# openMVG/openMVG

Hardware: AMD Instinct MI355X
Metric: descriptor pairs/s (brute-force L2 2-NN + ratio matching) (higher is better)
Workload: dtype i8 (int32 accumulate); 1 GPU; 1000 images x 2000 SIFT-like uint8x128 descriptors, exhaustive pairs (499500 image pairs, 499500 on rank 0), ratio 0.8; parallelism=pair-sharded x1, no collective

## Files before the change

### include/mvgx.h

```cpp
#ifndef MVGX_H_
#define MVGX_H_

#include <stddef.h>
#include <stdint.h>

#ifdef __cplusplus
extern "C" {
#endif

#define MVGX_OK 0
#define MVGX_ERR_ARG 1
#define MVGX_ERR_HIP 2
#define MVGX_ERR_NODEV 3
#define MVGX_ERR_STATE 4
#define MVGX_ERR_UNSUPPORTED 5
#define MVGX_ERR_NUMERIC 6
#define MVGX_ERR_STRUCTURE 7

const char* mvgx_last_error(void);
int mvgx_device_count(int* count);
int mvgx_abi_version(void);


typedef struct mvgx_match_ctx mvgx_match_ctx;
// ... 10 lines not shown
  uint32_t kernel_vgprs;
  uint32_t variant;
} mvgx_match_stats;

int mvgx_match_create(int device, mvgx_match_ctx** out);
int mvgx_match_create_multi(const int* devices, int n_devices, mvgx_match_ctx** out);
int mvgx_match_destroy(mvgx_match_ctx* ctx);

int mvgx_match_set_option(mvgx_match_ctx* ctx, const char* key, int64_t value);

int mvgx_match_set_regions(mvgx_match_ctx* ctx, const uint8_t* const* desc_rows, const uint32_t* n_desc,
                           uint32_t n_images, uint32_t dim);

int mvgx_match_set_regions_device(mvgx_match_ctx* ctx, const void* d_desc_concat, const uint32_t* n_desc,
                                  uint32_t n_images, uint32_t dim);

int mvgx_match_run(mvgx_match_ctx* ctx, const uint32_t* pairs_IJ, uint64_t n_pairs, float ratio_sq,
                   mvgx_match_stats* stats );

typedef int (*mvgx_match_batch_sink)(void* user, uint64_t first_pair, uint32_t n_pairs, const uint32_t* offsets,
                                     const uint32_t* ij);
int mvgx_match_run_stream(mvgx_match_ctx* ctx, const uint32_t* pairs_IJ, uint64_t n_pairs, float ratio_sq,
                          mvgx_match_batch_sink sink, void* user, mvgx_match_stats* stats );

int mvgx_match_results(mvgx_match_ctx* ctx, const uint64_t** offsets, const uint32_t** ij);

int mvgx_match_pairs_u8_l2(const uint8_t* const* desc_rows, const uint32_t* n_desc, uint32_t n_images,
                           uint32_t dim, const uint32_t* pairs_IJ, uint64_t n_pairs, float ratio_sq,
                           int device, mvgx_match_sink sink, void* user);

typedef struct mvgx_hamming_ctx mvgx_hamming_ctx;
int mvgx_hamming_create(int device, mvgx_hamming_ctx** out);
int mvgx_hamming_destroy(mvgx_hamming_ctx* ctx);
int mvgx_hamming_set_option(mvgx_hamming_ctx* ctx, const char* key , int64_t value);
int mvgx_hamming_set_regions(mvgx_hamming_ctx* ctx, const uint8_t* const* desc_rows, const uint32_t* n_desc,
                             uint32_t n_images, uint32_t desc_bytes);
int mvgx_hamming_run(mvgx_hamming_ctx* ctx, const uint32_t* pairs_IJ, uint64_t n_pairs, float dist_ratio,
                     mvgx_match_stats* stats );
int mvgx_hamming_results(mvgx_hamming_ctx* ctx, const uint64_t** offsets, const uint32_t** ij);

typedef struct mvgx_l2f_ctx mvgx_l2f_ctx;
int mvgx_l2f_create(int device, mvgx_l2f_ctx** out);
int mvgx_l2f_destroy(mvgx_l2f_ctx* ctx);
int mvgx_l2f_set_option(mvgx_l2f_ctx* ctx, const char* key , int64_t value);
int mvgx_l2f_set_regions(mvgx_l2f_ctx* ctx, const float* const* desc_rows, const uint32_t* n_desc, uint32_t n_images,
                         uint32_t dim);
// ... 273 lines not shown
```

### openmvg_amd/_capi.py

```python
import ctypes as C
import os

_HERE = os.path.dirname(os.path.abspath(__file__))
LIB_PATH = os.environ.get("MVGX_LIB_PATH") or os.path.join(_HERE, "lib", "libmvgx_hip.so")

MVGX_OK = 0
MVGX_ERR_ARG, MVGX_ERR_HIP, MVGX_ERR_NODEV, MVGX_ERR_STATE, MVGX_ERR_UNSUPPORTED, MVGX_ERR_NUMERIC, MVGX_ERR_STRUCTURE = 1, 2, 3, 4, 5, 6, 7
MVGX_BA_MAX_INTR_PARAMS = 8


class MvgxError(RuntimeError):
    def __init__(self, code, msg):
        super().__init__(f"mvgx error {code}: {msg}")
        self.code = code


class MatchStats(C.Structure):
    _fields_ = [
        ("n_pairs", C.c_uint64),
        ("n_desc_pairs", C.c_uint64),
        ("n_matches", C.c_uint64),
        ("n_kernel_launches", C.c_uint64),
        ("kernel_ms", C.c_double),
        ("total_ms", C.c_double),
# ... 117 lines not shown
class ResectionOptions(C.Structure):
    _fields_ = [("solver", C.c_int32), ("max_iteration", C.c_uint32), ("error_max", C.c_double), ("waves_ahead", C.c_uint32),
                ("global_above", C.c_uint32)]


class ResectionStats(C.Structure):
    _fields_ = [("n_problems", C.c_uint64), ("n_iterations", C.c_uint64), ("n_models", C.c_uint64), ("kernel_ms", C.c_double),
                ("total_ms", C.c_double)]


PROTOTYPES = {
    "mvgx_last_error": (C.c_char_p, []),
    "mvgx_device_count": (C.c_int, [C.POINTER(C.c_int)]),
    "mvgx_abi_version": (C.c_int, []),
    "mvgx_match_create": (C.c_int, [C.c_int, C.POINTER(C.c_void_p)]),
    "mvgx_match_create_multi": (C.c_int, [C.POINTER(C.c_int), C.c_int, C.POINTER(C.c_void_p)]),
    "mvgx_match_destroy": (C.c_int, [C.c_void_p]),
    "mvgx_match_set_option": (C.c_int, [C.c_void_p, C.c_char_p, C.c_int64]),
    "mvgx_match_set_regions": (C.c_int, [C.c_void_p, C.POINTER(C.c_void_p), C.POINTER(C.c_uint32), C.c_uint32, C.c_uint32]),
    "mvgx_match_set_regions_device": (C.c_int, [C.c_void_p, C.c_void_p, C.POINTER(C.c_uint32), C.c_uint32, C.c_uint32]),
    "mvgx_match_run": (C.c_int, [C.c_void_p, C.c_void_p, C.c_uint64, C.c_float, C.POINTER(MatchStats)]),
    "mvgx_match_run_stream": (C.c_int, [C.c_void_p, C.c_void_p, C.c_uint64, C.c_float, MATCH_BATCH_SINK, C.c_void_p,
                                        C.POINTER(MatchStats)]),
    "mvgx_match_results": (C.c_int, [C.c_void_p, C.POINTER(C.POINTER(C.c_uint64)), C.POINTER(C.POINTER(C.c_uint32))]),
    "mvgx_match_pairs_u8_l2": (C.c_int, [C.POINTER(C.c_void_p), C.POINTER(C.c_uint32), C.c_uint32, C.c_uint32, C.c_void_p,
                                          C.c_uint64, C.c_float, C.c_int, MATCH_SINK, C.c_void_p]),
    "mvgx_hamming_create": (C.c_int, [C.c_int, C.POINTER(C.c_void_p)]),
    "mvgx_hamming_destroy": (C.c_int, [C.c_void_p]),
    "mvgx_hamming_set_option": (C.c_int, [C.c_void_p, C.c_char_p, C.c_int64]),
    "mvgx_hamming_set_regions": (C.c_int, [C.c_void_p, C.POINTER(C.c_void_p), C.POINTER(C.c_uint32), C.c_uint32, C.c_uint32]),
    "mvgx_hamming_run": (C.c_int, [C.c_void_p, C.c_void_p, C.c_uint64, C.c_float, C.POINTER(MatchStats)]),
    "mvgx_hamming_results": (C.c_int, [C.c_void_p, C.POINTER(C.POINTER(C.c_uint64)), C.POINTER(C.POINTER(C.c_uint32))]),
    "mvgx_l2f_create": (C.c_int, [C.c_int, C.POINTER(C.c_void_p)]),
    "mvgx_l2f_destroy": (C.c_int, [C.c_void_p]),
    "mvgx_l2f_set_option": (C.c_int, [C.c_void_p, C.c_char_p, C.c_int64]),
    "mvgx_l2f_set_regions": (C.c_int, [C.c_void_p, C.POINTER(C.c_void_p), C.POINTER(C.c_uint32), C.c_uint32, C.c_uint32]),
    "mvgx_l2f_run": (C.c_int, [C.c_void_p, C.c_void_p, C.c_uint64, C.c_float, C.POINTER(MatchStats)]),
    "mvgx_l2f_results": (C.c_int, [C.c_void_p, C.POINTER(C.POINTER(C.c_uint64)), C.POINTER(C.POINTER(C.c_uint32))]),
    "mvgx_l2u8_create": (C.c_int, [C.c_int, C.POINTER(C.c_void_p)]),
    "mvgx_l2u8_destroy": (C.c_int, [C.c_void_p]),
    "mvgx_l2u8_set_option": (C.c_int, [C.c_void_p, C.c_char_p, C.c_int64]),
    "mvgx_l2u8_set_regions": (C.c_int, [C.c_void_p, C.POINTER(C.c_void_p), C.POINTER(C.c_uint32), C.c_uint32, C.c_uint32]),
    "mvgx_l2u8_run": (C.c_int, [C.c_void_p, C.c_void_p, C.c_uint64, C.c_float, C.POINTER(MatchStats)]),
    "mvgx_l2u8_results": (C.c_int, [C.c_void_p, C.POINTER(C.POINTER(C.c_uint64)), C.POINTER(C.POINTER(C.c_uint32))]),
    "mvgx_cascade_create": (C.c_int, [C.c_int, C.POINTER(C.c_void_p)]),
    "mvgx_cascade_destroy": (C.c_int, [C.c_void_p]),
# ... 98 lines not shown
```

### openmvg_amd/csrc/mvgx_match.hip

```cpp
#include <hip/hip_runtime.h>

#include <algorithm>
#include <atomic>
#include <climits>
#include <condition_variable>
#include <cstdint>
#include <cstdlib>
#include <cstring>
#include <functional>
#include <mutex>
#include <string>
#include <thread>
#include <vector>

#include "mvgx_buffers.h"
#include "mvgx_common.h"
#include "mvgx_match_batch.h"

namespace {

using mvgx::DevBuf;
using mvgx::PinnedBuf;
using mvgx::set_error;

// ... 1175 lines not shown
      const uint32_t* dbr = reinterpret_cast<const uint32_t*>(rowsI + (size_t)i * kDim);
      int d = 0;
#pragma unroll
      for (int k = 0; k < 32; ++k) {
        const uint32_t x = qv[k], y = dbr[k];
#pragma unroll
        for (int bb = 0; bb < 4; ++bb) {
          const int df = (int)((x >> (8 * bb)) & 0xFF) - (int)((y >> (8 * bb)) & 0xFF);
          d += df * df;
        }
      }
      if (d < d0) { d1 = d0; d0 = d; i0 = i; }
      else if (d < d1) { d1 = d; }
    }
    const bool ok = __int2float_rn(d0) < __fmul_rn(p.ratio_sq, __int2float_rn(d1));
    p.best[(size_t)wk.x * p.qstride + p.rowpos[p.img_row_off[J] + q]] = ok ? i0 : kNoMatch;
    if (ok) atomicAdd(&p.count[wk.x], 1u);
  }
}


}

struct mvgx_match_ctx {
  int device = 0;
  hipStream_t stream = nullptr;
  hipEvent_t ev_total0 = nullptr, ev_total1 = nullptr;
  int variant = 4;
  int filter_shape = 16;
  int stage = 3;
  int profile = 0;
  int64_t batch_pairs = 1 << 15;
  int keep_host_results = 1;
  int overlap = 1;
  int verify_alone = 0;
  int debug_filter = 0;
  int stream_hold = 0;
  int pinned_stream = 1;
  uint32_t n_images = 0;
  uint32_t total_tiles = 0;
  uint32_t max_tiles_pad = 0;
  uint32_t qstride = 0;
  std::vector<uint32_t> h_n, h_tile_off, h_ntiles;
  std::vector<uint32_t> h_qtile_off;
  std::vector<uint64_t> h_row_off;
  DevBuf<uint8_t> d_rows;
  bool rows_owned = true;
  const uint8_t* d_rows_view = nullptr;
  DevBuf<int8_t> d_tiles, d_rows_slot, d_qtiles;
  DevBuf<int> d_rconst, d_cinit, d_qnorm, d_rownorm, d_qtnorm;
  DevBuf<uint64_t> d_row_off;
  DevBuf<uint32_t> d_tile_off, d_qtile_off, d_n, d_ntiles, d_perm, d_rowpos, d_neven, d_err;
  struct Slot {
    hipStream_t stream = nullptr;
    hipEvent_t ev_scan = nullptr;
    hipEvent_t ev_filter = nullptr;
    DevBuf<uint2> d_pairs, d_work, d_ij;
    DevBuf<uint4> d_work8, d_work8h;
    DevBuf<uint32_t> d_best, d_count, d_offsets;
    DevBuf<int2> d_cd;
    PinnedBuf<uint2> hp_pairs, hp_work;
    PinnedBuf<uint4> hp_work8, hp_work8h;
    PinnedBuf<uint32_t> hp_offsets;
    uint64_t p0 = 0;
    uint32_t nb = 0;
    hipEvent_t ev_copy = nullptr;
    PinnedBuf<uint32_t> hp_ij[2];
    std::vector<uint32_t> h_off_out[2];
    int out_set = 0;
    uint64_t out_p0 = 0;
    uint32_t out_nb = 0;
  } slot[2];
  struct Results {
    std::vector<uint64_t> offsets;
    PinnedBuf<uint32_t> ij;
    size_t ij_n = 0;
  } results[2];
  int cur = 0;
  int double_buffer = 0;
  std::vector<hipEvent_t> ev_pool;
  std::vector<mvgx_match_ctx*> children;
};

namespace {

enum WorkList { kListItems16 = 0, kListItems8h = 1, kListRecords = 2 };
using MatchKernel = void (*)(MatchParams);
struct KernelForm {
// ... 37 lines not shown
    for (uint32_t qt = 0; qt < c->h_ntiles[J]; qt += kBlockQTiles) out[n++] = make_uint2(k, qt);
  }
  return n;
}
uint32_t build_items8h(const mvgx_match_ctx* c, const uint32_t* ij, uint32_t nb, uint4* out) {
  uint32_t n = 0;
  for (uint32_t k = 0; k < nb; ++k) {
    const uint32_t I = ij[2 * k], J = ij[2 * k + 1];
    if (!pair_has_work(c, I, J)) continue;
    for (uint32_t qt = 0; qt < c->h_ntiles[J]; qt += kBlockQTilesH) {
      out[2 * n] = make_uint4(k, qt, c->h_tile_off[I], c->h_tile_off[J]);
      out[2 * n + 1] = make_uint4(c->h_ntiles[I], c->h_tile_off[J + 1] - c->h_tile_off[J], 0, 0);
      ++n;
    }
  }
  return n;
}
uint32_t build_records(const mvgx_match_ctx* c, const uint32_t* ij, uint32_t nb, uint4* out) {
  const mvgx_records::ImageTables im{c->h_n.data(), c->h_tile_off.data(), c->h_ntiles.data(), c->h_qtile_off.data()};
  return mvgx_records::build_block_records(im, ij, nb, reinterpret_cast<uint32_t*>(out));
}

template <typename T>
int upload_list(DevBuf<T>& d, const PinnedBuf<T>& h, size_t n, hipStream_t stream) {
  const int rc = d.ensure(std::max<size_t>(n, 1));
  if (rc) return rc;
  if (n) MVGX_HIP(hipMemcpyAsync(d.p, h.p, n * sizeof(T), hipMemcpyHostToDevice, stream));
  return MVGX_OK;
}

int prep_regions(mvgx_match_ctx* c) {
  const uint32_t n_images = c->n_images;
  c->h_tile_off.assign(n_images + 1, 0);
  c->h_row_off.assign(n_images + 1, 0);
  c->h_ntiles.assign(n_images + 1, 0);
  c->h_qtile_off.assign(n_images + 1, 0);
  uint32_t max_n = 0;
  for (uint32_t k = 0; k < n_images; ++k) {
    c->h_row_off[k + 1] = c->h_row_off[k] + c->h_n[k];
    c->h_qtile_off[k + 1] = c->h_qtile_off[k] + (c->h_n[k] + kTileRows - 1) / kTileRows;
    max_n = std::max(max_n, c->h_n[k]);
  }
  const uint64_t total_rows = c->h_row_off[n_images];
  int rc;
  if ((rc = c->d_row_off.ensure(n_images + 1))) return rc;
  if ((rc = c->d_tile_off.ensure(n_images + 1))) return rc;
  if ((rc = c->d_qtile_off.ensure(n_images + 1))) return rc;
  if ((rc = c->d_n.ensure(n_images + 1))) return rc;
// ... 172 lines not shown
}

int mvgx_match_set_option(mvgx_match_ctx* c, const char* key, int64_t value) {
  MVGX_REQUIRE(c && key, MVGX_ERR_ARG, "mvgx_match_set_option: NULL argument");
  if (strcmp(key, "pinned_results") && strcmp(key, "double_buffer_results") && strcmp(key, "keep_host_results"))
    for (mvgx_match_ctx* child : c->children) {
      const int rc = mvgx_match_set_option(child, key, value);
      if (rc) return rc;
    }
  if (!strcmp(key, "variant")) {
    MVGX_REQUIRE(value >= 0 && value <= 4, MVGX_ERR_ARG, "variant must be 0..4");
    c->variant = (int)value;
  } else if (!strcmp(key, "filter_shape")) {
    MVGX_REQUIRE(value == 16 || value == 17 || value == 32, MVGX_ERR_ARG, "filter_shape must be 16, 17 (16x16x64, three workgroups per CU) or 32");
    c->filter_shape = (int)value;
  } else if (!strcmp(key, "stage")) {
    MVGX_REQUIRE(value >= 1 && value <= 3, MVGX_ERR_ARG, "stage must be 1..3");
    c->stage = (int)value;
  } else if (!strcmp(key, "profile")) {
    c->profile = value < 0 ? 0 : (int)std::min<int64_t>(value, 2);
  } else if (!strcmp(key, "batch_pairs")) {
    MVGX_REQUIRE(value >= 1 && value <= (1 << 20), MVGX_ERR_ARG, "batch_pairs must be in [1, 2^20]");
    c->batch_pairs = value;
  } else if (!strcmp(key, "keep_host_results")) {
    c->keep_host_results = value != 0;
  } else if (!strcmp(key, "overlap")) {
    c->overlap = value != 0;
  } else if (!strcmp(key, "verify_alone")) {
    c->verify_alone = value != 0;
  } else if (!strcmp(key, "debug_filter")) {
    MVGX_REQUIRE(value == 0 || value == 8 || value == 16, MVGX_ERR_ARG,
                 "debug_filter must be 0, 8 or 16 (the epilogue forms of l2_filter_kernel: window fold, both partitions per chain, "
                 "window fold with a single-buffered initialiser)");
    c->debug_filter = (int)value;
  } else if (!strcmp(key, "stream_hold")) {
    c->stream_hold = value != 0;
  } else if (!strcmp(key, "pinned_stream")) {
    c->pinned_stream = value != 0;
  } else if (!strcmp(key, "stream_reserve")) {
    MVGX_REQUIRE(value >= 0 && value <= (int64_t)1 << 31, MVGX_ERR_ARG, "stream_reserve: words per buffer in [0, 2^31]");
    if (c->pinned_stream && value > 0) {
      MVGX_HIP(hipSetDevice(c->device));
      for (auto& sl : c->slot)
        for (int set = 0; set < (c->stream_hold ? 2 : 1); ++set) {
          PinnedBuf<uint32_t>& hb = sl.hp_ij[set];
          if (!hb.p) hb.pageable = false;
// ... 56 lines not shown
}

int mvgx_match_set_regions_device(mvgx_match_ctx* c, const void* d_desc_concat, const uint32_t* n_desc,
                                  uint32_t n_images, uint32_t dim) {
  MVGX_REQUIRE(c && n_desc && (d_desc_concat || n_images == 0), MVGX_ERR_ARG,
               "mvgx_match_set_regions_device: NULL argument");
  MVGX_REQUIRE(dim == kDim, MVGX_ERR_UNSUPPORTED, "descriptor length %u unsupported (device path is 128-D uint8)", dim);
  MVGX_REQUIRE(c->children.empty(), MVGX_ERR_UNSUPPORTED, "mvgx_match_set_regions_device: a device pointer belongs to one device; "
               "use mvgx_match_set_regions on a multi-device context");
  MVGX_HIP(hipSetDevice(c->device));
  c->n_images = n_images;
  c->h_n.assign(n_desc, n_desc + n_images);
  c->rows_owned = false;
  c->d_rows_view = static_cast<const uint8_t*>(d_desc_concat);
  return prep_regions(c);
}

}

namespace {

struct BatchFeed {
  const uint32_t* pairs_IJ = nullptr;
  uint64_t n_pairs = 0, B = 1;
  std::atomic<uint64_t> next{0};
  std::atomic<int> stop{0};
  bool take(uint64_t& p0, uint32_t& nb) {
    if (stop.load(std::memory_order_relaxed)) return false;
    p0 = next.fetch_add(B);
    if (p0 >= n_pairs) return false;
    nb = (uint32_t)std::min<uint64_t>(B, n_pairs - p0);
    return true;
  }
};

using BatchSink = std::function<int(uint64_t p0, uint32_t nb, const uint32_t* offsets, const uint32_t* ij)>;

int run_device(mvgx_match_ctx* c, BatchFeed& feed, float ratio_sq, const BatchSink* sink, mvgx_match_stats& st) {
  const uint32_t* pairs_IJ = feed.pairs_IJ;
  MVGX_HIP(hipSetDevice(c->device));
  mvgx_match_ctx::Results& res = c->results[c->cur];
  memset(&st, 0, sizeof(st));
  st.variant = (uint32_t)c->variant;
  size_t n_ev = 0;
  int rc;

  MVGX_HIP(hipEventRecord(c->ev_total0, c->slot[0].stream));

  const KernelForm form = resolve_form(c);
  auto issue = [&](mvgx_match_ctx::Slot& sl, mvgx_match_ctx::Slot* prev, uint64_t p0, uint32_t nb) -> int {
    int rc;
    hipStream_t stream = sl.stream;
    sl.p0 = p0; sl.nb = nb;
    const uint32_t* ij = pairs_IJ + 2 * p0;
    if ((rc = sl.hp_pairs.ensure(nb))) return rc;
    for (uint32_t k = 0; k < nb; ++k) {
      const uint32_t I = ij[2 * k], J = ij[2 * k + 1];
      sl.hp_pairs.p[k] = make_uint2(I, J);
      if (!pair_has_work(c, I, J)) continue;
      st.n_pairs += 1;
      st.n_desc_pairs += (uint64_t)c->h_n[I] * c->h_n[J];
    }
    const size_t max_items16 = (size_t)nb * std::max<uint32_t>(1, (c->max_tiles_pad + kBlockQTiles - 1) / kBlockQTiles);
    uint32_t n_list[3] = {0, 0, 0};
    if (form.reads(kListItems16)) {
      if ((rc = sl.hp_work.ensure(max_items16))) return rc;
      n_list[kListItems16] = build_items16(c, ij, nb, sl.hp_work.p);
    }
    if (form.reads(kListItems8h)) {
      if ((rc = sl.hp_work8h.ensure(max_items16 * 4))) return rc;
      n_list[kListItems8h] = build_items8h(c, ij, nb, sl.hp_work8h.p);
    }
    if (form.reads(kListRecords)) {
      if ((rc = sl.hp_work8.ensure(max_items16 * kRecQuads))) return rc;
      n_list[kListRecords] = build_records(c, ij, nb, sl.hp_work8.p);
    }
    const uint32_t n_filter = n_list[form.list], n_verify = n_list[form.verify_list];
    if ((rc = sl.d_pairs.ensure(nb))) return rc;
    if ((rc = sl.d_best.ensure((size_t)nb * c->qstride))) return rc;
    if (form.verify && (rc = sl.d_cd.ensure((size_t)nb * c->qstride))) return rc;
    if ((rc = sl.d_count.ensure(nb))) return rc;
    if ((rc = sl.d_offsets.ensure((size_t)nb + 1))) return rc;
    if ((rc = sl.hp_offsets.ensure((size_t)nb + 1))) return rc;
    MVGX_HIP(hipMemcpyAsync(sl.d_pairs.p, sl.hp_pairs.p, nb * sizeof(uint2), hipMemcpyHostToDevice, stream));
    if (form.reads(kListItems16) && (rc = upload_list(sl.d_work, sl.hp_work, n_list[kListItems16], stream))) return rc;
    if (form.reads(kListItems8h) && (rc = upload_list(sl.d_work8h, sl.hp_work8h, (size_t)n_list[kListItems8h] * 2, stream))) return rc;
    if (form.reads(kListRecords) && (rc = upload_list(sl.d_work8, sl.hp_work8, (size_t)n_list[kListRecords] * kRecQuads, stream))) return rc;
    MVGX_HIP(hipMemsetAsync(sl.d_count.p, 0, nb * sizeof(uint32_t), stream));

    MatchParams mp;
    mp.tiles = c->d_tiles.p; mp.rows_slot = c->d_rows_slot.p; mp.rconst = c->d_rconst.p; mp.cinit = c->d_cinit.p; mp.qnorm = c->d_qnorm.p;
    mp.perm = c->d_perm.p; mp.rowpos = c->d_rowpos.p; mp.qtiles = c->d_qtiles.p; mp.qtnorm = c->d_qtnorm.p;
    mp.rows_u8 = c->d_rows_view; mp.img_row_off = c->d_row_off.p;
    mp.img_tile_off = c->d_tile_off.p; mp.img_n = c->d_n.p; mp.img_ntiles = c->d_ntiles.p;
    mp.cd = sl.d_cd.p; mp.img_neven = c->d_neven.p; mp.errflag = c->d_err.p;
    mp.pairs = sl.d_pairs.p; mp.work = sl.d_work.p; mp.work8 = sl.d_work8.p; mp.work8h = sl.d_work8h.p; mp.n_work = n_filter;
    mp.best = sl.d_best.p; mp.count = sl.d_count.p; mp.qstride = c->qstride; mp.ratio_sq = ratio_sq;

    if (prev) MVGX_HIP(hipStreamWaitEvent(stream, prev->ev_filter, 0));
    if (n_filter) {
      hipEvent_t e0 = nullptr, e1 = nullptr;
      if (c->profile) {
        e0 = get_event(c, n_ev++); e1 = get_event(c, n_ev++);
        MVGX_REQUIRE(e0 && e1, MVGX_ERR_HIP, "hipEventCreate failed");
        MVGX_HIP(hipEventRecord(e0, stream));
      }
      hipLaunchKernelGGL(form.filter, dim3(n_filter), dim3(256), form.lds_bytes, stream, mp);
      MVGX_HIP(hipGetLastError());
      if (c->profile) MVGX_HIP(hipEventRecord(e1, stream));
      if (!c->verify_alone) MVGX_HIP(hipEventRecord(sl.ev_filter, stream));
// ... 16 lines not shown
    uint32_t* const d_offsets = sl.d_offsets.p;
    hipLaunchKernelGGL(scan_counts_kernel, dim3(1), dim3(1024), 0, stream, mp.count, nb, d_offsets);
    MVGX_HIP(hipGetLastError());
    MVGX_HIP(hipMemcpyAsync(sl.hp_offsets.p, sl.d_offsets.p, ((size_t)nb + 1) * sizeof(uint32_t), hipMemcpyDeviceToHost, stream));
    MVGX_HIP(hipEventRecord(sl.ev_scan, stream));
    return MVGX_OK;
  };
  auto finish = [&](mvgx_match_ctx::Slot& sl) -> int {
    int rc;
    MVGX_HIP(hipEventSynchronize(sl.ev_scan));
    const uint32_t nb = sl.nb;
    const uint64_t p0 = sl.p0;
    const uint32_t total = sl.hp_offsets.p[nb];
    if (sink) {
      if (c->stream_hold) sl.out_set ^= 1;
      sl.h_off_out[sl.out_set].assign(sl.hp_offsets.p, sl.hp_offsets.p + nb + 1);
    } else {
      const uint64_t base = res.offsets[p0];
      for (uint32_t k = 0; k <= nb; ++k) res.offsets[p0 + k] = base + sl.hp_offsets.p[k];
    }
    sl.out_p0 = p0; sl.out_nb = nb;
    st.n_matches += total;
    if (total) {
      if ((rc = sl.d_ij.ensure(total))) return rc;
      hipStream_t stream = sl.stream;
      const uint32_t *d_best = sl.d_best.p, *d_offsets = sl.d_offsets.p;
      const uint2* d_pairs = sl.d_pairs.p;
      uint2* d_ij = sl.d_ij.p;
      hipLaunchKernelGGL(compact_matches_kernel, dim3((nb + 3) / 4), dim3(256), 0, stream, d_best, d_offsets, d_pairs, c->d_n.p,
                         c->d_row_off.p, form.dense_slots ? nullptr : c->d_rowpos.p, nb, c->qstride, d_ij);
      MVGX_HIP(hipGetLastError());
      if (sink) {
        PinnedBuf<uint32_t>& hb = sl.hp_ij[sl.out_set];
        if (!hb.p) hb.pageable = !c->pinned_stream;
        if ((size_t)total * 2 > hb.cap) { hb.release(); if ((rc = hb.grow_keep(std::max<size_t>((size_t)total * 3, 4u << 20), 0))) return rc; }
        MVGX_HIP(hipMemcpyAsync(hb.p, sl.d_ij.p, (size_t)total * sizeof(uint2), hipMemcpyDeviceToHost, sl.stream));
      } else if (c->keep_host_results) {
        const size_t old = res.ij_n;
        if (old + (size_t)total * 2 > res.ij.cap)
          for (auto& o : c->slot) MVGX_HIP(hipStreamSynchronize(o.stream));
        if ((rc = res.ij.grow_keep(old + (size_t)total * 2, old))) return rc;
        res.ij_n = old + (size_t)total * 2;
        MVGX_HIP(hipMemcpyAsync(res.ij.p + old, sl.d_ij.p, (size_t)total * sizeof(uint2),
                                hipMemcpyDeviceToHost, sl.stream));
      }
    }
    if (sink) MVGX_HIP(hipEventRecord(sl.ev_copy, sl.stream));
    return MVGX_OK;
  };
  auto deliver = [&](mvgx_match_ctx::Slot& sl) -> int {
    MVGX_HIP(hipEventSynchronize(sl.ev_copy));
    if (feed.stop.load()) return MVGX_OK;
    if ((*sink)(sl.out_p0, sl.out_nb, sl.h_off_out[sl.out_set].data(), sl.hp_ij[sl.out_set].p)) feed.stop.store(1);
    return MVGX_OK;
  };
  uint64_t nbatch = 0, p0 = 0;
  uint32_t nb = 0;
  while (feed.take(p0, nb)) {
    mvgx_match_ctx::Slot& cur = c->slot[nbatch & 1];
    mvgx_match_ctx::Slot* prev = nbatch ? &c->slot[(nbatch - 1) & 1] : nullptr;
    if (!c->overlap) {
      if ((rc = issue(cur, nullptr, p0, nb)) || (rc = finish(cur))) return rc;
      MVGX_HIP(hipStreamSynchronize(cur.stream));
      if (sink && (rc = deliver(cur))) return rc;
      ++nbatch;
      continue;
    }
    if ((rc = issue(cur, prev, p0, nb))) return rc;
    if (prev && (rc = finish(*prev))) return rc;
    if (sink && nbatch >= 2 && (rc = deliver(cur))) return rc;
    ++nbatch;
  }
  if (c->overlap && nbatch) {
    mvgx_match_ctx::Slot& last = c->slot[(nbatch - 1) & 1];
    if (sink && nbatch >= 2 && (rc = deliver(c->slot[nbatch & 1]))) return rc;
    if ((rc = finish(last))) return rc;
    if (sink && (rc = deliver(last))) return rc;
  }
  for (auto& sl : c->slot) MVGX_HIP(hipStreamSynchronize(sl.stream));
  MVGX_HIP(hipEventRecord(c->ev_total1, c->slot[0].stream));
  MVGX_HIP(hipEventSynchronize(c->ev_total1));
  float ms = 0.f;
  MVGX_HIP(hipEventElapsedTime(&ms, c->ev_total0, c->ev_total1));
  st.total_ms = ms;
  if (form.verify) {
    uint32_t flags[2] = {0, 0};
    MVGX_HIP(hipMemcpy(flags, c->d_err.p, 2 * sizeof(uint32_t), hipMemcpyDeviceToHost));
    (void)hipMemset(c->d_err.p, 0, 2 * sizeof(uint32_t));
    const uint32_t nerr = flags[0];
    st.kernel_vgprs = flags[1];
    if (nerr) {
// ... 85 lines not shown
  MVGX_REQUIRE(c && (pairs_IJ || n_pairs == 0), MVGX_ERR_ARG, "%s: NULL argument", who);
  const mvgx_match_ctx* r = c->children.empty() ? c : c->children[0];
  MVGX_REQUIRE(r->d_rows_view != nullptr || r->n_images == 0, MVGX_ERR_STATE, "%s before set_regions", who);
  const int rc = check_ratio(ratio_sq, "ratio_sq");
  return rc ? rc : check_pairs_in_range(pairs_IJ, n_pairs, r->n_images, who);
}

uint64_t batch_size(const mvgx_match_ctx* c) {
  return batch_size(c->batch_pairs, (c->children.empty() ? c : c->children[0])->qstride);
}

}

extern "C" {

int mvgx_match_run(mvgx_match_ctx* c, const uint32_t* pairs_IJ, uint64_t n_pairs, float ratio_sq,
                   mvgx_match_stats* stats) {
  int rc = check_run_args(c, pairs_IJ, n_pairs, ratio_sq, "mvgx_match_run");
  if (rc) return rc;
  if (c->double_buffer) c->cur ^= 1;
  mvgx_match_ctx::Results& res = c->results[c->cur];
  res.offsets.assign(n_pairs + 1, 0);
  res.ij_n = 0;
  BatchFeed feed;
  feed.pairs_IJ = pairs_IJ; feed.n_pairs = n_pairs; feed.B = batch_size(c);
  mvgx_match_stats st;
  if (c->children.empty()) {
    rc = run_device(c, feed, ratio_sq, nullptr, st);
  } else {
    struct Piece { uint64_t p0; std::vector<uint32_t> ij; };
    std::vector<Piece> pieces;
    BatchSink collect = [&](uint64_t p0, uint32_t nb, const uint32_t* offsets, const uint32_t* ij) -> int {
      for (uint32_t k = 0; k < nb; ++k) res.offsets[p0 + k + 1] = offsets[k + 1] - offsets[k];
      if (c->keep_host_results && offsets[nb]) pieces.push_back(Piece{p0, std::vector<uint32_t>(ij, ij + 2 * (size_t)offsets[nb])});
      return 0;
    };
    rc = run_multi(c, feed, ratio_sq, collect, st);
    if (rc == MVGX_OK) {
      for (uint64_t k = 0; k < n_pairs; ++k) res.offsets[k + 1] += res.offsets[k];
      if (c->keep_host_results) {
        if ((rc = res.ij.grow_keep(2 * res.offsets[n_pairs], 0))) return rc;
        res.ij_n = 2 * res.offsets[n_pairs];
        for (const Piece& p : pieces) memcpy(res.ij.p + 2 * res.offsets[p.p0], p.ij.data(), p.ij.size() * sizeof(uint32_t));
      }
    }
  }
  if (rc == MVGX_OK && stats) *stats = st;
  return rc;
}

int mvgx_match_run_stream(mvgx_match_ctx* c, const uint32_t* pairs_IJ, uint64_t n_pairs, float ratio_sq,
                          mvgx_match_batch_sink sink, void* user, mvgx_match_stats* stats) {
  int rc = check_run_args(c, pairs_IJ, n_pairs, ratio_sq, "mvgx_match_run_stream");
  if (rc) return rc;
  MVGX_REQUIRE(sink != nullptr, MVGX_ERR_ARG, "mvgx_match_run_stream: sink is NULL");
  BatchFeed feed;
  feed.pairs_IJ = pairs_IJ; feed.n_pairs = n_pairs; feed.B = batch_size(c);
  BatchSink fn = [&](uint64_t p0, uint32_t nb, const uint32_t* offsets, const uint32_t* ij) -> int {
    return sink(user, p0, nb, offsets, ij);
  };
  mvgx_match_stats st;
  rc = c->children.empty() ? run_device(c, feed, ratio_sq, &fn, st) : run_multi(c, feed, ratio_sq, fn, st);
  if (rc == MVGX_OK && stats) *stats = st;
  return rc;
}

int mvgx_match_results(mvgx_match_ctx* c, const uint64_t** offsets, const uint32_t** ij) {
  MVGX_REQUIRE(c && offsets && ij, MVGX_ERR_ARG, "mvgx_match_results: NULL argument");
  *offsets = c->results[c->cur].offsets.data();
  *ij = c->results[c->cur].ij.p;
  return MVGX_OK;
}

int mvgx_match_pairs_u8_l2(const uint8_t* const* desc_rows, const uint32_t* n_desc, uint32_t n_images,
                           uint32_t dim, const uint32_t* pairs_IJ, uint64_t n_pairs, float ratio_sq, int device,
                           mvgx_match_sink sink, void* user) {
  mvgx_match_ctx* c = nullptr;
  int rc = mvgx_match_create(device, &c);
  if (rc) return rc;
  rc = mvgx_match_set_regions(c, desc_rows, n_desc, n_images, dim);
  if (!rc) rc = mvgx_match_run(c, pairs_IJ, n_pairs, ratio_sq, nullptr);
  if (!rc && sink) {
    for (uint64_t k = 0; k < n_pairs; ++k) {
      const uint64_t a = c->results[c->cur].offsets[k], b = c->results[c->cur].offsets[k + 1];
      if (b > a) sink(user, pairs_IJ[2 * k], pairs_IJ[2 * k + 1], c->results[c->cur].ij.p + 2 * a, (uint32_t)(b - a));
    }
  }
// ... 6 lines not shown
```

### openmvg_amd/csrc/mvgx_match_batch.h

```cpp
#pragma once
#include <cstddef>
#include <cstdint>

namespace mvgx_records {

constexpr int kRecWaves = 4;
constexpr int kUnitBlocks = 8;
constexpr int kBlockRows = 16;
constexpr int kRecQuads = 1 + 2 * kRecWaves;

struct ImageTables {
  const uint32_t* n;
  const uint32_t* tile_off;
  const uint32_t* ntiles;
  const uint32_t* qtile_off;
};

inline bool pair_has_work(const uint32_t* n, uint32_t I, uint32_t J) { return n[I] >= 2 && n[J] != 0; }

inline uint32_t build_block_records(const ImageTables& im, const uint32_t* ij, uint32_t nb, uint32_t* out) {
  uint32_t n_rec = 0, rec_used = kRecWaves, unit_I = 0;
  uint32_t* unit = nullptr;
  uint32_t unit_blocks = 0, unit_segs = 0;
  for (uint32_t k = 0; k < nb; ++k) {
    const uint32_t I = ij[2 * k], J = ij[2 * k + 1];
    if (!pair_has_work(im.n, I, J)) continue;
    const uint32_t nblk = (im.n[J] + kBlockRows - 1) / kBlockRows;
    for (uint32_t blk = 0; blk < nblk;) {
      if (!unit || unit_I != I || unit_blocks == kUnitBlocks || unit_segs == 2) {
        if (rec_used == kRecWaves || unit_I != I) {
          uint32_t* r = out + (size_t)4 * kRecQuads * n_rec++;
          r[0] = im.tile_off[I]; r[1] = im.ntiles[I]; r[2] = 0; r[3] = 0;
          for (int q = 1; q < kRecQuads; ++q) { r[4 * q] = 0; r[4 * q + 1] = im.qtile_off[I]; r[4 * q + 2] = 0; r[4 * q + 3] = 0; }
          rec_used = 0;
        }
        unit = out + (size_t)4 * kRecQuads * (n_rec - 1) + 4 * (1 + 2 * rec_used++);
        unit_I = I; unit_blocks = 0; unit_segs = 0;
      }
      const uint32_t take = (nblk - blk < kUnitBlocks - unit_blocks) ? nblk - blk : kUnitBlocks - unit_blocks;
      uint32_t* seg = unit + 4 * unit_segs;
      seg[0] = k; seg[1] = im.qtile_off[J]; seg[3] = im.n[J];
      if (unit_segs == 0) { seg[2] = blk; unit[4 + 2] = take; }
      ++unit_segs; unit_blocks += take; blk += take;
    }
  }
  return n_rec;
}

}

#ifndef MVGX_MATCH_BATCH_RECORDS_ONLY
#include <hip/hip_runtime.h>

#include <algorithm>

#include "mvgx_common.h"

namespace {

constexpr uint32_t kNoMatch = 0xFFFFFFFFu;

__global__ __launch_bounds__(1024) void scan_counts_kernel(const uint32_t* __restrict__ count, uint32_t n,
                                                           uint32_t* __restrict__ offsets ) {
  __shared__ uint32_t s_part[1024];
  const uint32_t per = (n + 1023) / 1024;
  const uint32_t lo = min(n, threadIdx.x * per), hi = min(n, lo + per);
  uint32_t sum = 0;
  for (uint32_t i = lo; i < hi; ++i) sum += count[i];
  s_part[threadIdx.x] = sum;
// ... 63 lines not shown
```

### openmvg_amd/matching.py

```python
import ctypes as C
from enum import IntEnum

import numpy as np

from . import _capi


class EMatcherType(IntEnum):
    BRUTE_FORCE_L2 = 0
    ANN_L2 = 1
    CASCADE_HASHING_L2 = 2
    HNSW_L2 = 3
    HNSW_L1 = 4
    BRUTE_FORCE_HAMMING = 5
    HNSW_HAMMING = 6


def exhaustivePairs(N):
    return [(i, j) for i in range(N) for j in range(i + 1, N)]


def contiguousWithOverlap(N, overlapSize):
    return [(i, j) for i in range(N) for j in range(i + 1, min(i + 1 + overlapSize, N))]

# ... 139 lines not shown
    def run_stream(self, pairs, ratio_sq, on_batch=None):
        pairs = np.ascontiguousarray(pairs, dtype=np.uint32).reshape(-1, 2)
        st = _capi.MatchStats()
        err = []

        def sink(_user, first_pair, nb, offsets, ij):
            if on_batch is None:
                return 0
            try:
                off = np.ctypeslib.as_array(offsets, shape=(nb + 1,))
                total = int(off[nb])
                lists = np.ctypeslib.as_array(ij, shape=(total, 2)) if total else np.zeros((0, 2), np.uint32)
                return 1 if on_batch(int(first_pair), off, lists) else 0
            except BaseException as e:
                err.append(e)
                return 1

        cb = _capi.MATCH_BATCH_SINK(sink)
        _capi.check(_capi.lib().mvgx_match_run_stream(self._h, pairs.ctypes.data, pairs.shape[0], np.float32(ratio_sq), cb, None,
                                                      C.byref(st)))
        if err:
            raise err[0]
        return st

    def run_collect_stream(self, pairs, ratio_sq):
        pairs = np.ascontiguousarray(pairs, dtype=np.uint32).reshape(-1, 2)
        counts = np.zeros(len(pairs) + 1, np.uint64)
        pieces = {}

        def on_batch(p0, off, lists):
            counts[p0 + 1:p0 + len(off)] = np.diff(off.astype(np.int64)).astype(np.uint64)
            pieces[p0] = lists.copy()

        st = self.run_stream(pairs, ratio_sq, on_batch)
        offsets = np.cumsum(counts, dtype=np.uint64)
        keys = sorted(pieces)
        ij = np.concatenate([pieces[k] for k in keys]) if keys else np.zeros((0, 2), np.uint32)
        return st, offsets, ij, keys


class HammingContext:
    _prefix = "mvgx_hamming"
    _dtype = np.uint8

    def _fn(self, name):
        return getattr(_capi.lib(), f"{self._prefix}_{name}")
# ... 296 lines not shown
```

Measured before the change: 10670 billion descriptor pairs/s.

## Ramp batch sizes at pipeline edges and sort records by query-tile chunk per XCD

Replaces fixed-size batching with a schedule whose first and last batches are smaller (B/8, B/4, B/2), so the double-buffered host/device pipeline fills and drains sooner. Device and pinned buffers are reserved for the largest batch up front to avoid reallocation as sizes ramp. It also reorders work records on the host with a counting sort keyed on query-tile chunk, within each of 8 per-XCD slices, so records that touch the same query data run together for cache reuse. The cost is extra host-side sorting per batch and more kernel launches at the ramps. A batch-schedule query API is added.

```diff
diff --git a/include/mvgx.h b/include/mvgx.h
--- a/include/mvgx.h
+++ b/include/mvgx.h
@@ -56,6 +56,9 @@
                                      const uint32_t* ij);
 int mvgx_match_run_stream(mvgx_match_ctx* ctx, const uint32_t* pairs_IJ, uint64_t n_pairs, float ratio_sq,
                           mvgx_match_batch_sink sink, void* user, mvgx_match_stats* stats );
+
+int mvgx_match_batch_schedule(mvgx_match_ctx* ctx, uint64_t n_pairs, uint64_t* first_pair, uint32_t* batch_pairs, uint64_t capacity,
+                              uint64_t* n_batches);
 
 int mvgx_match_results(mvgx_match_ctx* ctx, const uint64_t** offsets, const uint32_t** ij);
 
diff --git a/openmvg_amd/_capi.py b/openmvg_amd/_capi.py
--- a/openmvg_amd/_capi.py
+++ b/openmvg_amd/_capi.py
@@ -163,6 +163,7 @@
     "mvgx_match_run": (C.c_int, [C.c_void_p, C.c_void_p, C.c_uint64, C.c_float, C.POINTER(MatchStats)]),
     "mvgx_match_run_stream": (C.c_int, [C.c_void_p, C.c_void_p, C.c_uint64, C.c_float, MATCH_BATCH_SINK, C.c_void_p,
                                         C.POINTER(MatchStats)]),
+    "mvgx_match_batch_schedule": (C.c_int, [C.c_void_p, C.c_uint64, C.c_void_p, C.c_void_p, C.c_uint64, C.POINTER(C.c_uint64)]),
     "mvgx_match_results": (C.c_int, [C.c_void_p, C.POINTER(C.POINTER(C.c_uint64)), C.POINTER(C.POINTER(C.c_uint32))]),
     "mvgx_match_pairs_u8_l2": (C.c_int, [C.POINTER(C.c_void_p), C.POINTER(C.c_uint32), C.c_uint32, C.c_uint32, C.c_void_p,
                                           C.c_uint64, C.c_float, C.c_int, MATCH_SINK, C.c_void_p]),
diff --git a/openmvg_amd/csrc/mvgx_match.hip b/openmvg_amd/csrc/mvgx_match.hip
--- a/openmvg_amd/csrc/mvgx_match.hip
+++ b/openmvg_amd/csrc/mvgx_match.hip
@@ -1221,6 +1221,10 @@
 
 }
 
+#ifndef MVGX_MATCH_RECORD_ORDER
+#define MVGX_MATCH_RECORD_ORDER 1
+#endif
+
 struct mvgx_match_ctx {
   int device = 0;
   hipStream_t stream = nullptr;
@@ -1230,6 +1234,10 @@
   int stage = 3;
   int profile = 0;
   int64_t batch_pairs = 1 << 15;
+  int64_t batch_ramp = 1024;
+  int record_order = MVGX_MATCH_RECORD_ORDER;
+  int record_chunk_tiles = mvgx_records::kOrderChunkTiles;
+  std::vector<uint32_t> h_rec_tmp, h_rec_count;
   int keep_host_results = 1;
   int overlap = 1;
   int verify_alone = 0;
@@ -1262,7 +1270,7 @@
     PinnedBuf<uint4> hp_work8, hp_work8h;
     PinnedBuf<uint32_t> hp_offsets;
     uint64_t p0 = 0;
-    uint32_t nb = 0;
+    uint32_t nb = 0, cap = 0;
     hipEvent_t ev_copy = nullptr;
     PinnedBuf<uint32_t> hp_ij[2];
     std::vector<uint32_t> h_off_out[2];
@@ -1346,8 +1354,8 @@
 }
 
 template <typename T>
-int upload_list(DevBuf<T>& d, const PinnedBuf<T>& h, size_t n, hipStream_t stream) {
-  const int rc = d.ensure(std::max<size_t>(n, 1));
+int upload_list(DevBuf<T>& d, const PinnedBuf<T>& h, size_t n, hipStream_t stream, size_t reserve = 0) {
+  const int rc = d.ensure(std::max<size_t>(std::max(n, reserve), 1));
   if (rc) return rc;
   if (n) MVGX_HIP(hipMemcpyAsync(d.p, h.p, n * sizeof(T), hipMemcpyHostToDevice, stream));
   return MVGX_OK;
@@ -1566,6 +1574,15 @@
   } else if (!strcmp(key, "batch_pairs")) {
     MVGX_REQUIRE(value >= 1 && value <= (1 << 20), MVGX_ERR_ARG, "batch_pairs must be in [1, 2^20]");
     c->batch_pairs = value;
+  } else if (!strcmp(key, "batch_ramp")) {
+    MVGX_REQUIRE(value >= 0 && value <= (1 << 20), MVGX_ERR_ARG, "batch_ramp must be in [0, 2^20] (pairs; 0: no ramps)");
+    c->batch_ramp = value;
+  } else if (!strcmp(key, "record_order")) {
+    MVGX_REQUIRE(value == 0 || value == 1, MVGX_ERR_ARG, "record_order must be 0 or 1");
+    c->record_order = (int)value;
+  } else if (!strcmp(key, "record_chunk_tiles")) {
+    MVGX_REQUIRE(value >= 1 && value <= (1 << 20), MVGX_ERR_ARG, "record_chunk_tiles must be in [1, 2^20]");
+    c->record_chunk_tiles = (int)value;
   } else if (!strcmp(key, "keep_host_results")) {
     c->keep_host_results = value != 0;
   } else if (!strcmp(key, "overlap")) {
@@ -1668,14 +1685,20 @@
 
 struct BatchFeed {
   const uint32_t* pairs_IJ = nullptr;
-  uint64_t n_pairs = 0, B = 1;
+  std::vector<mvgx_records::BatchSpan> batches;
+  uint32_t reserve_nb = 0;
   std::atomic<uint64_t> next{0};
   std::atomic<int> stop{0};
+  BatchFeed(const uint32_t* pairs, uint64_t n_pairs, uint64_t B, size_t nd, int64_t ramp_min) : pairs_IJ(pairs) {
+    batches = mvgx_records::batch_schedule(n_pairs, B, (uint32_t)std::max<size_t>(nd, 1), (uint64_t)ramp_min);
+    if (mvgx_records::batch_ramp_active(n_pairs, B, (uint64_t)ramp_min))
+      for (const auto& b : batches) reserve_nb = std::max(reserve_nb, b.nb);
+  }
   bool take(uint64_t& p0, uint32_t& nb) {
     if (stop.load(std::memory_order_relaxed)) return false;
-    p0 = next.fetch_add(B);
-    if (p0 >= n_pairs) return false;
-    nb = (uint32_t)std::min<uint64_t>(B, n_pairs - p0);
+    const uint64_t k = next.fetch_add(1);
+    if (k >= batches.size()) return false;
+    p0 = batches[k].p0; nb = batches[k].nb;
     return true;
   }
 };
@@ -1694,12 +1717,12 @@
   MVGX_HIP(hipEventRecord(c->ev_total0, c->slot[0].stream));
 
   const KernelForm form = resolve_form(c);
-  auto issue = [&](mvgx_match_ctx::Slot& sl, mvgx_match_ctx::Slot* prev, uint64_t p0, uint32_t nb) -> int {
+  auto issue = [&](mvgx_match_ctx::Slot& sl, mvgx_match_ctx::Slot* prev, uint64_t p0, uint32_t nb, uint32_t cap) -> int {
     int rc;
     hipStream_t stream = sl.stream;
-    sl.p0 = p0; sl.nb = nb;
+    sl.p0 = p0; sl.nb = nb; sl.cap = cap;
     const uint32_t* ij = pairs_IJ + 2 * p0;
-    if ((rc = sl.hp_pairs.ensure(nb))) return rc;
+    if ((rc = sl.hp_pairs.ensure(cap))) return rc;
     for (uint32_t k = 0; k < nb; ++k) {
       const uint32_t I = ij[2 * k], J = ij[2 * k + 1];
       sl.hp_pairs.p[k] = make_uint2(I, J);
@@ -1707,7 +1730,7 @@
       st.n_pairs += 1;
       st.n_desc_pairs += (uint64_t)c->h_n[I] * c->h_n[J];
     }
-    const size_t max_items16 = (size_t)nb * std::max<uint32_t>(1, (c->max_tiles_pad + kBlockQTiles - 1) / kBlockQTiles);
+    const size_t max_items16 = (size_t)cap * std::max<uint32_t>(1, (c->max_tiles_pad + kBlockQTiles - 1) / kBlockQTiles);
     uint32_t n_list[3] = {0, 0, 0};
     if (form.reads(kListItems16)) {
       if ((rc = sl.hp_work.ensure(max_items16))) return rc;
@@ -1719,19 +1742,27 @@
     }
     if (form.reads(kListRecords)) {
       if ((rc = sl.hp_work8.ensure(max_items16 * kRecQuads))) return rc;
-      n_list[kListRecords] = build_records(c, ij, nb, sl.hp_work8.p);
+      if (c->record_order) {
+        c->h_rec_tmp.resize(std::max(c->h_rec_tmp.size(), max_items16 * kRecQuads * 4));
+        n_list[kListRecords] = build_records(c, ij, nb, reinterpret_cast<uint4*>(c->h_rec_tmp.data()));
+        mvgx_records::order_records(c->h_qtile_off.data(), (uint32_t)c->record_chunk_tiles, ij, c->h_rec_tmp.data(), n_list[kListRecords],
+                                    reinterpret_cast<uint32_t*>(sl.hp_work8.p), c->h_rec_count);
+      } else {
+        n_list[kListRecords] = build_records(c, ij, nb, sl.hp_work8.p);
+      }
     }
     const uint32_t n_filter = n_list[form.list], n_verify = n_list[form.verify_list];
-    if ((rc = sl.d_pairs.ensure(nb))) return rc;
-    if ((rc = sl.d_best.ensure((size_t)nb * c->qstride))) return rc;
-    if (form.verify && (rc = sl.d_cd.ensure((size_t)nb * c->qstride))) return rc;
-    if ((rc = sl.d_count.ensure(nb))) return rc;
-    if ((rc = sl.d_offsets.ensure((size_t)nb + 1))) return rc;
-    if ((rc = sl.hp_offsets.ensure((size_t)nb + 1))) return rc;
+    if ((rc = sl.d_pairs.ensure(cap))) return rc;
+    if ((rc = sl.d_best.ensure((size_t)cap * c->qstride))) return rc;
+    if (form.verify && (rc = sl.d_cd.ensure((size_t)cap * c->qstride))) return rc;
+    if ((rc = sl.d_count.ensure(cap))) return rc;
+    if ((rc = sl.d_offsets.ensure((size_t)cap + 1))) return rc;
+    if ((rc = sl.hp_offsets.ensure((size_t)cap + 1))) return rc;
     MVGX_HIP(hipMemcpyAsync(sl.d_pairs.p, sl.hp_pairs.p, nb * sizeof(uint2), hipMemcpyHostToDevice, stream));
-    if (form.reads(kListItems16) && (rc = upload_list(sl.d_work, sl.hp_work, n_list[kListItems16], stream))) return rc;
-    if (form.reads(kListItems8h) && (rc = upload_list(sl.d_work8h, sl.hp_work8h, (size_t)n_list[kListItems8h] * 2, stream))) return rc;
-    if (form.reads(kListRecords) && (rc = upload_list(sl.d_work8, sl.hp_work8, (size_t)n_list[kListRecords] * kRecQuads, stream))) return rc;
+    const size_t res16 = cap > nb ? max_items16 : 0;
+    if (form.reads(kListItems16) && (rc = upload_list(sl.d_work, sl.hp_work, n_list[kListItems16], stream, res16))) return rc;
+    if (form.reads(kListItems8h) && (rc = upload_list(sl.d_work8h, sl.hp_work8h, (size_t)n_list[kListItems8h] * 2, stream, res16 * 4))) return rc;
+    if (form.reads(kListRecords) && (rc = upload_list(sl.d_work8, sl.hp_work8, (size_t)n_list[kListRecords] * kRecQuads, stream, res16 * kRecQuads))) return rc;
     MVGX_HIP(hipMemsetAsync(sl.d_count.p, 0, nb * sizeof(uint32_t), stream));
 
     MatchParams mp;
@@ -1794,7 +1825,8 @@
     sl.out_p0 = p0; sl.out_nb = nb;
     st.n_matches += total;
     if (total) {
-      if ((rc = sl.d_ij.ensure(total))) return rc;
+      const size_t total_cap = (size_t)((uint64_t)total * sl.cap / nb);
+      if (total > sl.d_ij.cap && (rc = sl.d_ij.ensure(total_cap))) return rc;
       hipStream_t stream = sl.stream;
       const uint32_t *d_best = sl.d_best.p, *d_offsets = sl.d_offsets.p;
       const uint2* d_pairs = sl.d_pairs.p;
@@ -1805,13 +1837,13 @@
       if (sink) {
         PinnedBuf<uint32_t>& hb = sl.hp_ij[sl.out_set];
         if (!hb.p) hb.pageable = !c->pinned_stream;
-        if ((size_t)total * 2 > hb.cap) { hb.release(); if ((rc = hb.grow_keep(std::max<size_t>((size_t)total * 3, 4u << 20), 0))) return rc; }
+        if ((size_t)total * 2 > hb.cap) { hb.release(); if ((rc = hb.grow_keep(std::max<size_t>(total_cap * 3, 4u << 20), 0))) return rc; }
         MVGX_HIP(hipMemcpyAsync(hb.p, sl.d_ij.p, (size_t)total * sizeof(uint2), hipMemcpyDeviceToHost, sl.stream));
       } else if (c->keep_host_results) {
         const size_t old = res.ij_n;
         if (old + (size_t)total * 2 > res.ij.cap)
           for (auto& o : c->slot) MVGX_HIP(hipStreamSynchronize(o.stream));
-        if ((rc = res.ij.grow_keep(old + (size_t)total * 2, old))) return rc;
+        if ((rc = res.ij.grow_keep(old + (old + (size_t)total * 2 > res.ij.cap ? total_cap : total) * 2, old))) return rc;
         res.ij_n = old + (size_t)total * 2;
         MVGX_HIP(hipMemcpyAsync(res.ij.p + old, sl.d_ij.p, (size_t)total * sizeof(uint2),
                                 hipMemcpyDeviceToHost, sl.stream));
@@ -1828,17 +1860,18 @@
   };
   uint64_t nbatch = 0, p0 = 0;
   uint32_t nb = 0;
+  auto slot_cap = [&](uint32_t nb) { return nbatch < 2 ? std::max(nb, feed.reserve_nb) : nb; };
   while (feed.take(p0, nb)) {
     mvgx_match_ctx::Slot& cur = c->slot[nbatch & 1];
     mvgx_match_ctx::Slot* prev = nbatch ? &c->slot[(nbatch - 1) & 1] : nullptr;
     if (!c->overlap) {
-      if ((rc = issue(cur, nullptr, p0, nb)) || (rc = finish(cur))) return rc;
+      if ((rc = issue(cur, nullptr, p0, nb, slot_cap(nb))) || (rc = finish(cur))) return rc;
       MVGX_HIP(hipStreamSynchronize(cur.stream));
       if (sink && (rc = deliver(cur))) return rc;
       ++nbatch;
       continue;
     }
-    if ((rc = issue(cur, prev, p0, nb))) return rc;
+    if ((rc = issue(cur, prev, p0, nb, slot_cap(nb)))) return rc;
     if (prev && (rc = finish(*prev))) return rc;
     if (sink && nbatch >= 2 && (rc = deliver(cur))) return rc;
     ++nbatch;
@@ -1970,8 +2003,7 @@
   mvgx_match_ctx::Results& res = c->results[c->cur];
   res.offsets.assign(n_pairs + 1, 0);
   res.ij_n = 0;
-  BatchFeed feed;
-  feed.pairs_IJ = pairs_IJ; feed.n_pairs = n_pairs; feed.B = batch_size(c);
+  BatchFeed feed(pairs_IJ, n_pairs, batch_size(c), c->children.size(), c->batch_ramp);
   mvgx_match_stats st;
   if (c->children.empty()) {
     rc = run_device(c, feed, ratio_sq, nullptr, st);
@@ -2002,8 +2034,7 @@
   int rc = check_run_args(c, pairs_IJ, n_pairs, ratio_sq, "mvgx_match_run_stream");
   if (rc) return rc;
   MVGX_REQUIRE(sink != nullptr, MVGX_ERR_ARG, "mvgx_match_run_stream: sink is NULL");
-  BatchFeed feed;
-  feed.pairs_IJ = pairs_IJ; feed.n_pairs = n_pairs; feed.B = batch_size(c);
+  BatchFeed feed(pairs_IJ, n_pairs, batch_size(c), c->children.size(), c->batch_ramp);
   BatchSink fn = [&](uint64_t p0, uint32_t nb, const uint32_t* offsets, const uint32_t* ij) -> int {
     return sink(user, p0, nb, offsets, ij);
   };
@@ -2011,6 +2042,18 @@
   rc = c->children.empty() ? run_device(c, feed, ratio_sq, &fn, st) : run_multi(c, feed, ratio_sq, fn, st);
   if (rc == MVGX_OK && stats) *stats = st;
   return rc;
+}
+
+int mvgx_match_batch_schedule(mvgx_match_ctx* c, uint64_t n_pairs, uint64_t* first_pair, uint32_t* batch_pairs, uint64_t capacity,
+                              uint64_t* n_batches) {
+  MVGX_REQUIRE(c && n_batches && ((first_pair && batch_pairs) || capacity == 0), MVGX_ERR_ARG, "mvgx_match_batch_schedule: NULL argument");
+  const BatchFeed feed(nullptr, n_pairs, batch_size(c), c->children.size(), c->batch_ramp);
+  *n_batches = feed.batches.size();
+  for (uint64_t k = 0; k < std::min<uint64_t>(capacity, feed.batches.size()); ++k) {
+    first_pair[k] = feed.batches[k].p0;
+    batch_pairs[k] = feed.batches[k].nb;
+  }
+  return MVGX_OK;
 }
 
 int mvgx_match_results(mvgx_match_ctx* c, const uint64_t** offsets, const uint32_t** ij) {
diff --git a/openmvg_amd/csrc/mvgx_match_batch.h b/openmvg_amd/csrc/mvgx_match_batch.h
--- a/openmvg_amd/csrc/mvgx_match_batch.h
+++ b/openmvg_amd/csrc/mvgx_match_batch.h
@@ -1,6 +1,8 @@
 #pragma once
 #include <cstddef>
 #include <cstdint>
+#include <cstring>
+#include <vector>
 
 namespace mvgx_records {
 
@@ -45,6 +47,71 @@
     }
   }
   return n_rec;
+}
+
+struct BatchSpan { uint64_t p0; uint32_t nb; };
+
+inline bool batch_ramp_active(uint64_t n_pairs, uint64_t B, uint64_t ramp_min) {
+  return ramp_min > 0 && B / 8 >= ramp_min && n_pairs >= 4 * B;
+}
+
+inline std::vector<BatchSpan> batch_schedule(uint64_t n_pairs, uint64_t B, uint32_t nd, uint64_t ramp_min) {
+  std::vector<BatchSpan> out;
+  if (B == 0) B = 1;
+  uint64_t p0 = 0;
+  auto put = [&](uint64_t nb) { out.push_back(BatchSpan{p0, (uint32_t)nb}); p0 += nb; };
+  if (!batch_ramp_active(n_pairs, B, ramp_min)) {
+    while (p0 < n_pairs) put(B < n_pairs - p0 ? B : n_pairs - p0);
+    return out;
+  }
+  const uint64_t steps[3] = {B / 8, B / 4, B / 2};
+  const uint64_t ramp = steps[0] + steps[1] + steps[2];
+  uint64_t rep = (n_pairs - B) / (2 * ramp);
+  if (rep > nd) rep = nd ? nd : 1;
+  const uint64_t mid = n_pairs - 2 * rep * ramp, n_mid = (mid + B - 1) / B;
+  for (int s = 0; s < 3; ++s)
+    for (uint64_t r = 0; r < rep; ++r) put(steps[s]);
+  for (uint64_t k = 0; k < n_mid; ++k) put(mid / n_mid + (k < mid % n_mid ? 1 : 0));
+  for (int s = 2; s >= 0; --s)
+    for (uint64_t r = 0; r < rep; ++r) put(steps[s]);
+  return out;
+}
+
+constexpr uint32_t kOrderChunkTiles = 256;
+
+inline void xcd_slice(uint32_t n_rec, uint32_t xcd, uint32_t& first, uint32_t& count) {
+  const uint32_t q = n_rec >> 3, r = n_rec & 7u;
+  first = xcd < r ? xcd * (q + 1) : r * (q + 1) + (xcd - r) * q;
+  count = q + (xcd < r ? 1 : 0);
+}
+
+inline uint32_t record_order_key(const uint32_t* qtile_off, uint32_t chunk_tiles, const uint32_t* ij, const uint32_t* rec) {
+  return qtile_off[ij[2 * rec[4] + 1]] / chunk_tiles;
+}
+
+inline void order_records(const uint32_t* qtile_off, uint32_t chunk_tiles, const uint32_t* ij, const uint32_t* src, uint32_t n_rec, uint32_t* dst,
+                          std::vector<uint32_t>& count) {
+  constexpr size_t kWords = (size_t)4 * kRecQuads;
+  for (uint32_t xcd = 0; xcd < 8; ++xcd) {
+    uint32_t first, n;
+    xcd_slice(n_rec, xcd, first, n);
+    if (!n) continue;
+    const uint32_t* s = src + kWords * first;
+    uint32_t* d = dst + kWords * first;
+    bool one_image = true;
+    uint32_t key_max = 0;
+    for (uint32_t k = 0; k < n; ++k) {
+      one_image = one_image && s[kWords * k] == s[0];
+      const uint32_t key = record_order_key(qtile_off, chunk_tiles, ij, s + kWords * k);
+      key_max = key > key_max ? key : key_max;
+    }
+    if (one_image) { std::memcpy(d, s, kWords * n * sizeof(uint32_t)); continue; }
+    count.assign((size_t)key_max + 2, 0);
+    for (uint32_t k = 0; k < n; ++k) ++count[record_order_key(qtile_off, chunk_tiles, ij, s + kWords * k) + 1];
+    for (uint32_t c = 0; c <= key_max; ++c) count[c + 1] += count[c];
+    for (uint32_t k = 0; k < n; ++k)
+      std::memcpy(d + kWords * count[record_order_key(qtile_off, chunk_tiles, ij, s + kWords * k)]++, s + kWords * k, kWords * sizeof(uint32_t));
+  }
 }
 
 }
diff --git a/openmvg_amd/matching.py b/openmvg_amd/matching.py
--- a/openmvg_amd/matching.py
+++ b/openmvg_amd/matching.py
@@ -185,6 +185,13 @@
         if err:
             raise err[0]
         return st
+
+    def batch_schedule(self, n_pairs):
+        n = C.c_uint64(0)
+        _capi.check(_capi.lib().mvgx_match_batch_schedule(self._h, int(n_pairs), None, None, 0, C.byref(n)))
+        first, nb = np.zeros(n.value, np.uint64), np.zeros(n.value, np.uint32)
+        _capi.check(_capi.lib().mvgx_match_batch_schedule(self._h, int(n_pairs), first.ctypes.data, nb.ctypes.data, n.value, C.byref(n)))
+        return [(int(a), int(b)) for a, b in zip(first, nb)]
 
     def run_collect_stream(self, pairs, ratio_sq):
         pairs = np.ascontiguousarray(pairs, dtype=np.uint32).reshape(-1, 2)
```

New measurement: 11030 billion descriptor pairs/s, median of 6. +3.4%, better.
